# swiss-territorial-data-lab/proj-roadsurf

Hardware: AMD Instinct MI355X
Metric: tiles_per_sec_512x512x3 (higher is better)
Workload: dtype f16 hi + lo operand planes (22 significand bits, 3 MFMA products per product) / f32 accumulate; 1 GPU; Mask R-CNN R50-FPN inference, batch 16 of 512x512 3-band tiles per GPU (BASELINE configs[1]), 800x800 network input; seeded synthetic weights, saturated: 1000 proposals and 100 detections per tile; batch_per_gpu=16, lanes=2, lane_streams=independent, num_classes=2, weights=random

## Files before the change

### proj_roadsurf_amd/csrc/common.h

```cpp
#pragma once
#include <hip/hip_runtime.h>
#include <stdint.h>
#include <stdio.h>

typedef _Float16 half_t;
typedef _Float16 half4 __attribute__((ext_vector_type(4)));
typedef _Float16 half8 __attribute__((ext_vector_type(8)));
typedef float f32x4 __attribute__((ext_vector_type(4)));

#define RS_OK 0
#define RS_ERR_ARG -1
#define RS_ERR_HIP -2
#define RS_ERR_BLOB -3
#define RS_ERR_UNSUPPORTED -4

void rs_set_error(const char* fmt, ...);

#define RS_HIP(expr)                                                                       \
  do {                                                                                     \
    hipError_t _e = (expr);                                                                \
    if (_e != hipSuccess) {                                                                \
      rs_set_error("%s:%d: %s -> %s", __FILE__, __LINE__, #expr, hipGetErrorString(_e));   \
      return RS_ERR_HIP;                                                                   \
    }                                                                                      \
  } while (0)

#define RS_CHECK(cond, code, ...)  \
  do {                             \
    if (!(cond)) {                 \
      rs_set_error(__VA_ARGS__);   \
      return (code);               \
    }                              \
  } while (0)

static inline int cdiv(long long a, long long b) { return (int)((a + b - 1) / b); }

#if defined(__HIPCC__)
__device__ __forceinline__ float rs_fdiv(float a, float b) {
  const float y0 = __builtin_amdgcn_rcpf(b);
  const float e = __builtin_fmaf(-b, y0, 1.0f);
  const float y = __builtin_fmaf(e, y0, y0);
  const float q0 = a * y;
  const float r0 = __builtin_fmaf(-b, q0, a);
  const float q1 = __builtin_fmaf(r0, y, q0);
  const float r1 = __builtin_fmaf(-b, q1, a);
  const float q = __builtin_fmaf(r1, y, q1);
  const bool special = !(__builtin_fabsf(b) > 0.f && __builtin_fabsf(b) < __builtin_inff() && __builtin_fabsf(a) > 0.f && __builtin_fabsf(a) < __builtin_inff());
  return special ? a * y0 : q;
}

__device__ __forceinline__ unsigned rs_sat_bad(float f) { return !(__builtin_fabsf(f) <= 65504.f); }
__device__ __forceinline__ void rs_sat_flush(unsigned long long* sat, unsigned cnt) {
  if (sat != nullptr && cnt != 0u) atomicAdd(sat, (unsigned long long)cnt);
}
#endif

struct RsDebug {
  int conv_single_stage_nk = 4;
  int conv_persist = 0;
  int conv_tuned = 1;
  int conv_deep = 1;
  int conv_wide_px = 128;
  int wreg_dbg = 0;
  int wreg_waves = 2;
  int conv_wreg = 1;
  int conv_wide1x1 = 1;
  int stem_small_tile = 1;
  int deep_dbg = 0;
  int deconv_variant = 22;
  int fuse_mask_predictor = 1;
  int side_stream = 1;
  int narrow_roialign = 0;
  int use_glds = 1;
  int fuse_shortcut = 1;
  int fuse_stem = 1;
  int fuse_bneck = 1;
  int deep_tile_px = 1;
  int deep_tail = 1;
  int fuse_rpn_heads = 1;
  int merge_levels = 1;
  int graph_small = 1;
  int use_graph = 0;
  int train_roi_side = -1;
  int train_side = -1;
  int wgrad_target = 512;
  int wgrad_cb = 0;
  int select_debug = 0;
  int nms_debug = 0;
  int roi_window = 1;
  int roi_bwd_atomic = 0;
  int roi_order = 1;
  int poly_edge_cap = 0;
  int poly_vertex_cap = 0;
};
const RsDebug& rs_debug();
void rs_debug_reload();

struct ConvSeg {
  const half_t* in;
  const half_t* w;
  const float* bias;
  void* out;
  float* head_out;
  int Ho, Wo, in_Hp, in_Wp, out_Hp, out_Wp;
  int M;
  int tile0;
  long long in_lo, out_lo;
  const float* wscale;
};
#define RS_MAX_SEGS 5

struct ConvParams {
  const half_t* in;
  const half_t* w;
  const float* bias;
  void* out;
  const half_t* res;
  const half_t* up;
  const int* m_count;
  const int* koff;
  int m_mul;
  int M;
  int Ho, Wo;
  int in_Hp, in_Wp, in_Cs, in_off;
  int stride;
  int KH, KW, Cin;
  int Kpad;
  int Cout;
  int out_Hp, out_Wp, out_Cs, out_pad;
  int up_Hp, up_Wp, up_Cs, up_pad;
  int relu;
  int mode;
  int out_f32;
  const float* dot_w;
// ... 180 lines not shown
```

### proj_roadsurf_amd/csrc/conv_deep.hip

```cpp
#include "conv_tile.h"

namespace {

constexpr int BN = 256, NT = 512, MI = 4, WCH = 4;
constexpr int ASTAGE = 256 * 128, WSTAGE = BN * 128;
constexpr int W_BASE = 3 * ASTAGE;
constexpr int LDS_BYTES = 3 * ASTAGE + 2 * WSTAGE;

template <int DBG, bool TRAIN, int NJ, bool SPLIT>
__device__ __forceinline__ void conv_deep_tile(const ConvParams& p, char* smem, const half_t* g_in, const half_t* g_w, const float* g_bias, void* g_out,
                                               float* g_head_out, const int Ho, const int Wo, const int in_Hp, const int in_Wp, const int out_Hp, const int out_Wp,
                                               const int M, const int m0, const int n0, const int q, const long long in_lo, const long long out_lo,
                                               const float* g_wscale) {
  constexpr int APS = (NJ + 1) / 2;
  constexpr int WPX = NJ * 16;
  const int tid = threadIdx.x;
  const int lane = tid & 63;
  const int wave = __builtin_amdgcn_readfirstlane(tid >> 6);
  const int wpx = wave / WCH, wch = wave % WCH;
  (void)q;

  const int lrow = lane >> 3, lchk = lane & 7;
  const half_t* aptr[APS];
  const half_t* wptr[4];
// ... 203 lines not shown
      } else {
        __builtin_amdgcn_sched_barrier(0);
        asm volatile("s_waitcnt lgkmcnt(0)" ::: "memory");
      }
      sab = snext;
      __builtin_amdgcn_sched_barrier(0);
#pragma unroll
      for (int i = 0; i < MI; ++i)
#pragma unroll
        for (int j = 0; j < NJ; ++j)
          acc[i][j] = __builtin_amdgcn_mfma_f32_16x16x32_f16(wf1[i], xf0[j], acc[i][j], 0, 0, 0);
    }
#undef RS_RD_W
#undef RS_RD_X
#ifdef RS_SPLIT_PHASES
    ph_loop1 = __builtin_amdgcn_s_memtime();
    if (p.probe && lane == 0) {
      long long* o = p.probe + ((long long)q * 8 + wave) * 8;
      o[0] = (long long)ph_work; o[1] = (long long)ph_vm; o[2] = (long long)ph_bar; o[3] = nk;
      o[4] = (long long)(ph_loop0 - ph_entry); o[5] = (long long)(ph_loop1 - ph_loop0);
    }
#endif
  } else {
  reads0(0, 0);
  int abuf = 0;
  for (int t = 0; t < nk; ++t) {
    __builtin_amdgcn_sched_barrier(0);
    reads1(abuf, t & 1);
    __builtin_amdgcn_sched_barrier(0);
    asm volatile("s_waitcnt lgkmcnt(%0)" ::"n"(4 + NJ) : "memory");
    __builtin_amdgcn_sched_barrier(0);
#pragma unroll
    for (int i = 0; i < MI; ++i)
#pragma unroll
      for (int j = 0; j < NJ; ++j)
        acc[i][j] = __builtin_amdgcn_mfma_f32_16x16x32_f16(wf0[i], xf0[j], acc[i][j], 0, 0, 0);
    __builtin_amdgcn_sched_barrier(0);
    const int anext = abuf == 2 ? 0 : abuf + 1;
    if (t + 1 < nk) {
      asm volatile("s_waitcnt lgkmcnt(0)" ::: "memory");
      if (t + 2 < nk) asm volatile("s_waitcnt vmcnt(%0)" ::"n"(APS) : "memory");
      else asm volatile("s_waitcnt vmcnt(0)" ::: "memory");
      asm volatile("s_barrier" ::: "memory");
      __builtin_amdgcn_sched_barrier(0);
#ifndef RS_DEEP_LOCKSTEP
      if (wpx) {
#pragma unroll
        for (int i = 0; i < MI; ++i)
#pragma unroll
          for (int j = 0; j < NJ; ++j)
            acc[i][j] = __builtin_amdgcn_mfma_f32_16x16x32_f16(wf1[i], xf1[j], acc[i][j], 0, 0, 0);
        __builtin_amdgcn_sched_barrier(0);
      }
#endif
      if (t + 2 < nk) stage_w();
      if (t + 3 < nk) stage_a();
      reads0(anext, (t + 1) & 1);
#ifndef RS_DEEP_LOCKSTEP
      if (wpx) { abuf = anext; continue; }
#endif
    }
    else {
      __builtin_amdgcn_sched_barrier(0);
      asm volatile("s_waitcnt lgkmcnt(0)" ::: "memory");
    }
    abuf = anext;
    __builtin_amdgcn_sched_barrier(0);
#pragma unroll
    for (int i = 0; i < MI; ++i)
#pragma unroll
      for (int j = 0; j < NJ; ++j)
        acc[i][j] = __builtin_amdgcn_mfma_f32_16x16x32_f16(wf1[i], xf1[j], acc[i][j], 0, 0, 0);
  }
  }

#ifdef RS_CLOCK_PROBE
  if (p.probe && tid == 0) {
    p.probe[2 * q] = (long long)(__builtin_amdgcn_s_memtime() - pr_t0);
    p.probe[2 * q + 1] = (long long)(__builtin_amdgcn_s_memrealtime() - pr_r0);
  }
#endif
  const int crow = n0 + wch * 64 + fq * 16;
  const EpiRows<MI, SPLIT> rw = epi_rows<MI, SPLIT>(g_bias, g_wscale, crow);
  unsigned satc = 0;
  if (!TRAIN && p.head_w) {
    const half_t* hw = p.head_w + (long long)fi * 256 + wch * 64 + fq * 8;
    const half8 ha0 = *(const half8*)hw, ha1 = *(const half8*)(hw + 32);
    half8 hl0, hl1;
    if constexpr (SPLIT) { hl0 = *(const half8*)(hw + p.head_w_lo); hl1 = *(const half8*)(hw + p.head_w_lo + 32); }
    f32x4 hacc[NJ];
#pragma unroll
    for (int j = 0; j < NJ; ++j) {
      half8 b0, b1, l0, l1;
      const bool mv = m0 + wpx * WPX + j * 16 + fi < M;
      unsigned sath = 0;
#pragma unroll
      for (int i = 0; i < MI; ++i)
#pragma unroll
        for (int r = 0; r < 4; ++r) {
          float f;
          if constexpr (SPLIT) f = acc[i][j][r] * rw.wsc[i * 4 + r] + rw.bias[i * 4 + r];
          else f = acc[i][j][r] + rw.bias[i * 4 + r];
          if (p.relu) f = f > 0.f ? f : 0.f;
          sath += mv ? rs_sat_bad(f) : 0u;
          const HiLo s = split_round(clamp_h16(f));
          if (i < 2) { b0[i * 4 + r] = s.h; l0[i * 4 + r] = s.l; } else { b1[(i - 2) * 4 + r] = s.h; l1[(i - 2) * 4 + r] = s.l; }
        }
      rs_sat_flush(p.sat, sath);
      f32x4 a = f32x4{0.f, 0.f, 0.f, 0.f};
      a = __builtin_amdgcn_mfma_f32_16x16x32_f16(ha0, b0, a, 0, 0, 0);
      a = __builtin_amdgcn_mfma_f32_16x16x32_f16(ha1, b1, a, 0, 0, 0);
      if constexpr (SPLIT) {
        a = __builtin_amdgcn_mfma_f32_16x16x32_f16(ha0, l0, a, 0, 0, 0);
        a = __builtin_amdgcn_mfma_f32_16x16x32_f16(ha1, l1, a, 0, 0, 0);
        a = __builtin_amdgcn_mfma_f32_16x16x32_f16(hl0, b0, a, 0, 0, 0);
        a = __builtin_amdgcn_mfma_f32_16x16x32_f16(hl1, b1, a, 0, 0, 0);
      }
      hacc[j] = a;
    }
    asm volatile("s_barrier" ::: "memory");
    float* part = (float*)smem;
#pragma unroll
    for (int j = 0; j < NJ; ++j) *(f32x4*)(part + ((wch * 2 * WPX + wpx * WPX + j * 16 + fi) * 16 + fq * 4)) = hacc[j];
    __syncthreads();
    const int px = tid >> 1, oh = (tid & 1) * 8;
    const int m = m0 + px;
    if (px < 2 * WPX && m < M) {
      f32x4 s0 = f32x4{0.f, 0.f, 0.f, 0.f}, s1 = f32x4{0.f, 0.f, 0.f, 0.f};
      if constexpr (!SPLIT) { s0 = *(const f32x4*)(p.head_b + oh); s1 = *(const f32x4*)(p.head_b + oh + 4); }
#pragma unroll
      for (int w = 0; w < 4; ++w) {
        s0 += *(const f32x4*)(part + ((w * 2 * WPX + px) * 16 + oh));
        s1 += *(const f32x4*)(part + ((w * 2 * WPX + px) * 16 + oh + 4));
      }
      if constexpr (SPLIT) {
        s0 = s0 * *(const f32x4*)(p.head_scale + oh) + *(const f32x4*)(p.head_b + oh);
        s1 = s1 * *(const f32x4*)(p.head_scale + oh + 4) + *(const f32x4*)(p.head_b + oh + 4);
      }
      const Pix hp = pix_of(m, Wo, Ho);
      float* op = g_head_out + ((long long)(hp.n * Ho + hp.y) * Wo + hp.x) * 16 + oh;
      *(f32x4*)op = s0;
      *(f32x4*)(op + 4) = s1;
    }
    return;
  }
#pragma unroll
  for (int j = 0; j < NJ; ++j) {
    const int m = m0 + wpx * WPX + j * 16 + fi;
    if (m >= M) continue;
    const Pix px = pix_of(m, Wo, Ho);
    const long long opix = (long long)(px.n * out_Hp + px.y + p.out_pad) * out_Wp + px.x + p.out_pad;
    float v[4 * MI];
    epi_values<MI, NJ, TRAIN, SPLIT>(v, p, acc, j, rw, opix, crow, px.x, px.y, px.n);
    if (p.out_f32) epi_store_f32<MI>((float*)g_out + opix * p.out_Cs + crow, v);
    else epi_store_h16<MI, SPLIT>((half_t*)g_out + opix * p.out_Cs + crow, out_lo, v, [&](float f, float) { satc += rs_sat_bad(f); });
  }
  rs_sat_flush(p.sat, satc);
#ifdef RS_SPLIT_PHASES
  if constexpr (SPLIT) {
    const unsigned long long ph_issued = __builtin_amdgcn_s_memtime();
    asm volatile("s_waitcnt vmcnt(0)" ::: "memory");
    const unsigned long long ph_drained = __builtin_amdgcn_s_memtime();
    if (p.probe && lane == 0) {
      long long* o = p.probe + ((long long)q * 8 + wave) * 8;
      o[6] = (long long)(ph_issued - ph_loop1); o[7] = (long long)(ph_drained - ph_issued);
    }
  }
#endif
}


template <int DBG, bool TRAIN = false, int NJF = 8, bool SPLIT = false>
__global__ __launch_bounds__(NT) void conv_deep_kernel(const ConvParams p) {
  constexpr int BM = 32 * NJF;
  extern __shared__ __attribute__((aligned(16))) char smem[];
  int M = conv_rows(p);
  const int tiles_n = p.Cout / BN;
  const int ntiles = p.nseg ? p.seg_tiles : tiles_n * ((M + BM - 1) / BM);
  const int nfull = ntiles - p.tail_tiles;
  const int q = blockIdx.x;
  if (q >= nfull + 2 * p.tail_tiles) return;
  const half_t* g_in = p.in;
  const half_t* g_w = p.w;
  const float* g_bias = p.bias;
  void* g_out = p.out;
  float* g_head_out = p.head_out;
  long long in_lo = p.in_lo, out_lo = p.out_lo;
  const float* g_wscale = p.wscale;
  int Ho = p.Ho, Wo = p.Wo, in_Hp = p.in_Hp, in_Wp = p.in_Wp, out_Hp = p.out_Hp, out_Wp = p.out_Wp;
  int L, half = -1;
  if (q < nfull) {
    L = xcd_tile(q, nfull);
  } else {
    L = nfull + ((q - nfull) >> 1);
    half = (q - nfull) & 1;
  }
  if (p.nseg) {
    int t0 = 0;
#pragma unroll
    for (int i = 0; i < RS_MAX_SEGS; ++i)
      if (i < p.nseg && L >= p.seg[i].tile0) {
        g_in = p.seg[i].in; g_w = p.seg[i].w; g_bias = p.seg[i].bias; g_out = p.seg[i].out; g_head_out = p.seg[i].head_out;
        Ho = p.seg[i].Ho; Wo = p.seg[i].Wo; in_Hp = p.seg[i].in_Hp; in_Wp = p.seg[i].in_Wp;
        out_Hp = p.seg[i].out_Hp; out_Wp = p.seg[i].out_Wp; M = p.seg[i].M; t0 = p.seg[i].tile0;
        if constexpr (SPLIT) { in_lo = p.seg[i].in_lo; out_lo = p.seg[i].out_lo; g_wscale = p.seg[i].wscale; }
      }
    L -= t0;
  }
  const int n0 = (L % tiles_n) * BN;
  const int m0 = (L / tiles_n) * BM;
  if (half < 0 || NJF != 8) {
    conv_deep_tile<DBG, TRAIN, NJF, SPLIT>(p, smem, g_in, g_w, g_bias, g_out, g_head_out, Ho, Wo, in_Hp, in_Wp, out_Hp, out_Wp, M, m0, n0, q, in_lo, out_lo, g_wscale);
  } else {
    if (m0 + half * (BM / 2) >= M) return;
    conv_deep_tile<DBG, TRAIN, NJF == 8 ? 4 : NJF, SPLIT>(p, smem, g_in, g_w, g_bias, g_out, g_head_out, Ho, Wo, in_Hp, in_Wp, out_Hp, out_Wp, M, m0 + half * (BM / 2), n0, q, in_lo, out_lo, g_wscale);
  }
}

}

int rs_device_cu_count() {
  static int ncu[64] = {0};
  int dev = 0;
  if (hipGetDevice(&dev) != hipSuccess || dev < 0 || dev >= 64) return 256;
  if (!ncu[dev]) {
    int n = 0;
    if (hipDeviceGetAttribute(&n, hipDeviceAttributeMultiprocessorCount, dev) != hipSuccess || n <= 0) n = 256;
    ncu[dev] = n;
  }
  return ncu[dev];
}

static int deep_tail_tiles(long long tiles) {
  const int ncu = rs_device_cu_count();
  if (!rs_debug().deep_tail) return 0;
  const int r = (int)(tiles % ncu);
  return (r > 0 && 2 * r <= ncu) ? r : 0;
}

static int no_scratch(const void* kernel, const char* what) {
// ... 146 lines not shown
```

### proj_roadsurf_amd/csrc/conv_igemm.hip

```cpp
#include "conv_tile.h"

namespace {

template <int WPX, int WCH, int MI, int NJ>
struct Tile {
  static constexpr int NW = WPX * WCH;
  static constexpr int NT = NW * 64;
  static constexpr int BM = WPX * NJ * 16;
  static constexpr int BN = WCH * MI * 16;
  static constexpr int STAGE = (BM + BN) * 128;
  static constexpr int LDS = 2 * STAGE + 1024;
};

template <int WPX, int WCH, int MI, int NJ, bool SMALLC, bool GLDS, bool PERSIST, bool TRAIN = false, bool SPLIT = false, bool FWD = false>
__global__ __launch_bounds__(WPX* WCH * 64) void conv_igemm_kernel(const ConvParams p) {
  using T = Tile<WPX, WCH, MI, NJ>;
  constexpr int NW = T::NW, BM = T::BM, BN = T::BN;
  constexpr int PA = BM / (NW * 8);
  constexpr int PW = (BN + NW * 8 - 1) / (NW * 8);
  extern __shared__ __attribute__((aligned(16))) char smem[];

  const int tid = threadIdx.x;
  const int lane = tid & 63;
  const int wave = __builtin_amdgcn_readfirstlane(tid >> 6);
// ... 147 lines not shown
      if (PERSIST && t == 0 && stores_in_flight) {
        if (stores_in_flight == NJ * STORES_F16) asm volatile("s_waitcnt vmcnt(%0)" ::"n"(NJ * STORES_F16) : "memory");
        else if (stores_in_flight == NJ * STORES_F32) asm volatile("s_waitcnt vmcnt(%0)" ::"n"(NJ * STORES_F32) : "memory");
        else asm volatile("s_waitcnt vmcnt(0)" ::: "memory");
        asm volatile("s_waitcnt lgkmcnt(0)" ::: "memory");
        __builtin_amdgcn_s_barrier();
      } else {
        asm volatile("s_waitcnt vmcnt(0)" ::: "memory");
        __syncthreads();
      }
      if (nst == 2) {
        if (t + 1 < nk) {
          stage((gs + 1) & 1, t + 1, SMALLC ? 0 : next_off());
        } else if (PERSIST && q + G < ntiles) {
          setup_tile(q + G);
          kh = 0; kw = 0; c0 = 0;
          stage((gs + 1) & 1, 0, SMALLC ? 0 : next_off());
        }
      }
      const char* sb = smem + (nst == 2 ? (gs & 1) : 0) * T::STAGE;
      if constexpr (SPLIT && !SMALLC) {
        half8 wh[MI], wl[MI], xh[NJ], xl[NJ];
#pragma unroll
        for (int i = 0; i < MI; ++i) { wh[i] = *(const half8*)(sb + w_off[i] + c0_off); wl[i] = *(const half8*)(sb + w_off[i] + c1_off); }
#pragma unroll
        for (int j = 0; j < NJ; ++j) { xh[j] = *(const half8*)(sb + x_off[j] + c0_off); xl[j] = *(const half8*)(sb + x_off[j] + c1_off); }
#pragma unroll
        for (int i = 0; i < MI; ++i)
#pragma unroll
          for (int j = 0; j < NJ; ++j) mfma_split3(acc[i][j], wh[i], wl[i], xh[j], xl[j]);
      } else if constexpr (NJ == 8) {
        half8 wf0[MI], xf0[NJ], wf1[MI], xf1[NJ];
#pragma unroll
        for (int i = 0; i < MI; ++i) wf0[i] = *(const half8*)(sb + w_off[i] + c0_off);
#pragma unroll
        for (int j = 0; j < NJ; ++j) xf0[j] = *(const half8*)(sb + x_off[j] + c0_off);
#pragma unroll
        for (int i = 0; i < MI; ++i) wf1[i] = *(const half8*)(sb + w_off[i] + c1_off);
#pragma unroll
        for (int j = 0; j < NJ; ++j) xf1[j] = *(const half8*)(sb + x_off[j] + c1_off);
#pragma unroll
        for (int i = 0; i < MI; ++i)
#pragma unroll
          for (int j = 0; j < NJ; ++j)
            acc[i][j] = __builtin_amdgcn_mfma_f32_16x16x32_f16(wf0[i], xf0[j], acc[i][j], 0, 0, 0);
#pragma unroll
        for (int i = 0; i < MI; ++i)
#pragma unroll
          for (int j = 0; j < NJ; ++j)
            acc[i][j] = __builtin_amdgcn_mfma_f32_16x16x32_f16(wf1[i], xf1[j], acc[i][j], 0, 0, 0);
      } else {
#pragma unroll
        for (int kk = 0; kk < 2; ++kk) {
          const int co = kk ? c1_off : c0_off;
          half8 wf[MI], xf[NJ];
#pragma unroll
          for (int i = 0; i < MI; ++i) wf[i] = *(const half8*)(sb + w_off[i] + co);
#pragma unroll
          for (int j = 0; j < NJ; ++j) xf[j] = *(const half8*)(sb + x_off[j] + co);
#pragma unroll
          for (int i = 0; i < MI; ++i)
#pragma unroll
            for (int j = 0; j < NJ; ++j)
              acc[i][j] = __builtin_amdgcn_mfma_f32_16x16x32_f16(wf[i], xf[j], acc[i][j], 0, 0, 0);
        }
      }
      if (nst == 1 && t + 1 < nk) {
        __syncthreads();
        stage(0, t + 1, SMALLC ? 0 : next_off());
      }
      ++gs;
    }

    const int ch_local = wch * MI * 16 + fq * 4 * MI;
    const int crow = n0c + ch_local;
    int g = 0, cb = crow;
    if (p.mode != 0) { g = crow / p.Cout; cb = crow % p.Cout; }
    constexpr bool DGRAD_SPLIT = TRAIN && SPLIT;
    constexpr bool FWD_SPLIT = DGRAD_SPLIT && FWD;
    const EpiRows<MI, SPLIT> rw = epi_rows<MI, SPLIT>(DGRAD_SPLIT && !FWD_SPLIT ? p.wscale : p.bias, p.wscale, crow);
    int e_dy = 0;
    if constexpr (FWD_SPLIT) e_dy = split_tensor_exp(p.x_amax[0], p.x_amax[1]);
    else if constexpr (DGRAD_SPLIT) e_dy = split_tensor_exp(p.dy_amax[0], p.dy_amax[1]);
    float dotp[NJ];
    long long dot_idx[NJ];
#pragma unroll
    for (int j = 0; j < NJ; ++j) { dotp[j] = 0.f; dot_idx[j] = -1; }
#pragma unroll
    for (int j = 0; j < NJ; ++j) {
      const int m = m0c + wpx * NJ * 16 + j * 16 + fi;
      if (m >= M) continue;
      const Pix px = pix_of(m, p.Wo, p.Ho);
      const int x = px.x, y = px.y, n = px.n;
      int oy = y, ox = x;
      if (p.mode != 0) { oy = 2 * y + (g >> 1); ox = 2 * x + (g & 1); }
      else if (TRAIN && p.out_stride > 1) { oy = y * p.out_stride; ox = x * p.out_stride; }
      const long long opix = (long long)(n * p.out_Hp + oy + p.out_pad) * p.out_Wp + ox + p.out_pad;
      float v[4 * MI];
      if constexpr (DGRAD_SPLIT) {
        if constexpr (FWD_SPLIT) epi_values_fwd_split<MI, NJ>(v, p, acc, j, rw, e_dy, opix, cb, x, y, n);
        else epi_values_dgrad_split<MI, NJ>(v, p, acc, j, rw, e_dy, opix, cb, x, y, n);
        epi_store_f32<MI>((float*)p.out + opix * p.out_Cs + cb, v);
        continue;
      } else {
        epi_values<MI, NJ, TRAIN, SPLIT>(v, p, acc, j, rw, opix, cb, x, y, n);
      }
      if (p.mode == 2) {
        const int slot = p.dot_slot[n];
        const float* wv = p.dot_w + (long long)p.dot_cls[slot] * p.Cout + cb;
        float sdot = 0.f;
#pragma unroll
        for (int i = 0; i < MI; ++i) {
          const f32x4 w4 = *(const f32x4*)(wv + i * 4);
#pragma unroll
          for (int r = 0; r < 4; ++r) sdot += v[i * 4 + r] * w4[r];
        }
        dotp[j] = sdot;
        dot_idx[j] = (long long)slot * (4 * p.Ho * p.Wo) + (long long)oy * (2 * p.Wo) + ox;
      } else if (p.out_f32) {
        epi_store_f32<MI>((float*)p.out + opix * p.out_Cs + cb, v);
      } else {
        float scr = 0.f;
        epi_store_h16<MI, SPLIT>((half_t*)p.out + opix * p.out_Cs + cb, p.out_lo, v, [&](float, float f) { scr += __builtin_fabsf(f); });
        if (!(scr < 65504.f)) {
          unsigned c = 0;
#pragma unroll
          for (int e = 0; e < 4 * MI; ++e) c += rs_sat_bad(v[e]);
          rs_sat_flush(p.sat, c);
        }
      }
    }
    if (p.mode == 2) {
      float* red = (float*)smem;
      __syncthreads();
#pragma unroll
      for (int j = 0; j < NJ; ++j) {
        float v0 = dotp[j];
        v0 += __shfl_xor(v0, 16);
        v0 += __shfl_xor(v0, 32);
        dotp[j] = v0;
        if (wch > 0 && fq == 0) red[(((wch - 1) * WPX + wpx) * NJ + j) * 16 + fi] = v0;
      }
      __syncthreads();
      if (wch == 0 && fq == 0) {
#pragma unroll
        for (int j = 0; j < NJ; ++j) {
          float v0 = dotp[j];
#pragma unroll
          for (int c = 1; c < WCH; ++c) v0 += red[(((c - 1) * WPX + wpx) * NJ + j) * 16 + fi];
          if (dot_idx[j] >= 0) atomicAdd(p.dot_out + dot_idx[j], v0);
        }
      }
    }

    stores_in_flight = (p.mode != 2 && m0c + BM <= M) ? NJ * (p.out_f32 ? STORES_F32 : STORES_F16) : 0;
    if constexpr (!PERSIST) break;
    q += G;
    if (q >= ntiles) break;
    if (nst == 1) {
      setup_tile(q);
      kh = 0; kw = 0; c0 = 0;
      __syncthreads();
      stage(0, 0, SMALLC ? 0 : next_off());
    }
  }
}

template <int WPX, int WCH, int MI, int NJ, bool SMALLC, bool CAN_PERSIST>
int launch_variant(const ConvParams& p, hipStream_t stream, int use_glds) {
  using T = Tile<WPX, WCH, MI, NJ>;
  const int rows = p.Cout * (p.mode != 0 ? 4 : 1);
  const int tiles_n = cdiv(rows, T::BN);
  const int tiles_m = cdiv(p.M, T::BM);
  const long long nblk = (long long)tiles_n * tiles_m;
  RS_CHECK(nblk > 0 && nblk < (1ll << 31), RS_ERR_ARG, "conv: bad grid %lld", nblk);
  RS_CHECK(rows % T::BN == 0 || T::BN <= 16, RS_ERR_ARG, "conv: Cout rows %d not a multiple of tile %d", rows, T::BN);
  const int lds = (p.stages == 1 ? 1 : 2) * T::STAGE + 1024;
  int bpc = CAN_PERSIST ? p.persist : 0;
  if (bpc < 0) bpc = (160 * 1024) / lds < 1 ? 1 : (160 * 1024) / lds;
  const bool persistent = bpc > 0 && p.stages != 1 && p.mode != 2 && use_glds && nblk > 256ll * bpc &&
                          !(p.down || p.res32 || p.mask || p.out_stride > 1);
  const bool train = p.down || p.res32 || p.mask || p.out_stride > 1;
  const void* k;
  if (p.split) {
    RS_CHECK(use_glds > 0 && !train && p.wscale, RS_ERR_UNSUPPORTED, "conv: the split-operand mode needs LDS-DMA staging, the row scales and no training epilogue");
    k = (const void*)conv_igemm_kernel<WPX, WCH, MI, NJ, SMALLC, true, false, false, true>;
  } else if (train) {
    RS_CHECK(use_glds && !SMALLC, RS_ERR_UNSUPPORTED, "conv: training epilogue options need LDS-DMA staging and Cin >= 64");
    if constexpr (!SMALLC) k = (const void*)conv_igemm_kernel<WPX, WCH, MI, NJ, false, true, false, true>;
    else k = nullptr;
  } else if constexpr (CAN_PERSIST) {
    k = persistent ? (const void*)conv_igemm_kernel<WPX, WCH, MI, NJ, SMALLC, true, true>
                   : (use_glds ? (const void*)conv_igemm_kernel<WPX, WCH, MI, NJ, SMALLC, true, false>
                               : (const void*)conv_igemm_kernel<WPX, WCH, MI, NJ, SMALLC, false, false>);
  } else {
    k = use_glds ? (const void*)conv_igemm_kernel<WPX, WCH, MI, NJ, SMALLC, true, false>
                 : (const void*)conv_igemm_kernel<WPX, WCH, MI, NJ, SMALLC, false, false>;
  }
  static bool attr[5] = {false, false, false, false, false};
  const int ai = p.split ? 4 : (train ? 3 : (persistent ? 2 : (use_glds ? 1 : 0)));
  if (!attr[ai]) {
    RS_HIP(hipFuncSetAttribute(k, hipFuncAttributeMaxDynamicSharedMemorySize, T::LDS));
    attr[ai] = true;
  }
  const unsigned grid = (persistent && !p.split) ? 256u * (unsigned)bpc : (unsigned)nblk;
  ConvParams pc = p;
  void* args[] = {&pc};
  RS_HIP(hipLaunchKernel(k, dim3(grid), dim3(T::NT), args, lds, stream));
  return RS_OK;
}

template <int WPX, int WCH, int MI, int NJ, bool FWD = false>
// ... 244 lines not shown
```

### proj_roadsurf_amd/csrc/conv_tile.h

```cpp
#pragma once
#include <stdint.h>

#if defined(__HIPCC__)
#include "common.h"
#define CT_D __device__ __forceinline__
#else
#define CT_D inline
#endif

CT_D int xcd_tile(int q, int n) {
  const int qn = n >> 3, r = n & 7, x = q & 7;
  return (x < r ? x * (qn + 1) : r * (qn + 1) + (x - r) * qn) + (q >> 3);
}

CT_D int act_key(int row) { return row & 7; }
CT_D int w_key(int row, int blk) { return (row & 3) | ((int)(((unsigned)row / (unsigned)blk) & 1u) << 2); }
CT_D int src_chunk(int lchk, int key) { return lchk ^ key; }
CT_D int chunk_f16(int d) { return d * 8; }
CT_D long long chunk_split(int d, long long lo) { return (d & 3) * 8 + (d >> 2) * lo; }
CT_D int frag_row(int fi, int i, int blk) { return (fi >> 2) * blk + i * 4 + (fi & 3); }
CT_D int frag_off(int fq, int fkey, int kk) { return ((4 * kk + fq) ^ fkey) * 16; }

struct Pix { int x, y, n; };
CT_D Pix pix_of(int m, int Wo, int Ho) {
  const int t = m / Wo;
  return Pix{m % Wo, t % Ho, t / Ho};
}
CT_D Pix pix_add(int x0, int y0, int n0, int rx, int ry, int rn, int Wo, int Ho) {
  int x = x0 + rx;
  const int cx = x >= Wo;
  x -= cx ? Wo : 0;
  int y = y0 + ry + cx;
  const int cy = y >= Ho;
  y -= cy ? Ho : 0;
  return Pix{x, y, n0 + rn + cy};
}

#if !defined(CT_NO_F16)
#if !defined(__HIPCC__)
typedef _Float16 half_t;
#endif
CT_D float clamp_h16(float f) { return f > 65504.f ? 65504.f : (f < -65504.f ? -65504.f : f); }
CT_D float clamp_h16_pos(float f) { return f > 65504.f ? 65504.f : f; }
struct HiLo { half_t h, l; };
CT_D HiLo split_round(float f) {
  const half_t h = (half_t)f;
  return HiLo{h, (half_t)(f - (float)h)};
}
#endif

#if defined(__HIPCC__)
__device__ __forceinline__ void glds16(const half_t* g, char* lds_wave_base) {
  __builtin_amdgcn_global_load_lds((const __attribute__((address_space(1))) void*)g,
                                   (__attribute__((address_space(3))) void*)lds_wave_base, 16, 0, 0);
}

template <class P>
__device__ __forceinline__ int conv_rows(const P& p) {
  int M = p.M;
  if (p.m_count) {
    const long long mc = (long long)(*p.m_count) * p.m_mul;
    if (mc < M) M = (int)mc;
  }
  return M;
}

__device__ __forceinline__ void mfma_split3(f32x4& acc, const half8& wh, const half8& wl, const half8& xh, const half8& xl) {
  acc = __builtin_amdgcn_mfma_f32_16x16x32_f16(wh, xl, acc, 0, 0, 0);
  acc = __builtin_amdgcn_mfma_f32_16x16x32_f16(wh, xh, acc, 0, 0, 0);
  acc = __builtin_amdgcn_mfma_f32_16x16x32_f16(wl, xh, acc, 0, 0, 0);
}

__device__ __forceinline__ int split_tensor_exp(unsigned amax_bits, unsigned nonfinite) {
  if (nonfinite || amax_bits == 0) return 0;
  const int be = (int)(amax_bits >> 23);
  const int E = be ? be - 127 : (31 - __clz((int)amax_bits)) - 149;
  return 14 - E;
}

template <int MI, bool SPLIT>
struct EpiRows {
  float bias[4 * MI];
  float wsc[SPLIT ? 4 * MI : 1];
};
template <int MI, bool SPLIT>
__device__ __forceinline__ EpiRows<MI, SPLIT> epi_rows(const float* bias, const float* wscale, int crow) {
  EpiRows<MI, SPLIT> rw;
#pragma unroll
  for (int i = 0; i < MI; ++i) {
    const f32x4 b4 = *(const f32x4*)(bias + crow + i * 4);
    rw.bias[i * 4 + 0] = b4[0]; rw.bias[i * 4 + 1] = b4[1]; rw.bias[i * 4 + 2] = b4[2]; rw.bias[i * 4 + 3] = b4[3];
  }
  if constexpr (SPLIT) {
#pragma unroll
    for (int i = 0; i < MI; ++i) {
      const f32x4 s4 = *(const f32x4*)(wscale + crow + i * 4);
      rw.wsc[i * 4 + 0] = s4[0]; rw.wsc[i * 4 + 1] = s4[1]; rw.wsc[i * 4 + 2] = s4[2]; rw.wsc[i * 4 + 3] = s4[3];
    }
  }
  return rw;
}

template <int MI, int NJ, bool TRAIN, bool SPLIT>
__device__ __forceinline__ void epi_values(float (&v)[4 * MI], const ConvParams& p, const f32x4 (&acc)[MI][NJ], const int j, const EpiRows<MI, SPLIT>& rw,
                                           const long long opix, const int cb, const int x, const int y, const int n) {
#pragma unroll
  for (int i = 0; i < MI; ++i)
#pragma unroll
    for (int r = 0; r < 4; ++r) {
      if constexpr (SPLIT) v[i * 4 + r] = acc[i][j][r] * rw.wsc[i * 4 + r] + rw.bias[i * 4 + r];
      else v[i * 4 + r] = acc[i][j][r] + rw.bias[i * 4 + r];
    }
  auto add_h16 = [&](const half_t* a, const long long lo) {
#pragma unroll
    for (int i = 0; i < MI; ++i) {
      const half4 h = *(const half4*)(a + i * 4);
      if constexpr (SPLIT) {
        const half4 l = *(const half4*)(a + lo + i * 4);
#pragma unroll
        for (int r = 0; r < 4; ++r) v[i * 4 + r] += (float)h[r] + (float)l[r];
      } else {
#pragma unroll
        for (int r = 0; r < 4; ++r) v[i * 4 + r] += (float)h[r];
      }
    }
  };
  if (p.res) add_h16(p.res + opix * p.out_Cs + cb, p.res_lo);
  if (p.up) {
    const long long upix = (long long)(n * p.up_Hp + (y >> 1) + p.up_pad) * p.up_Wp + (x >> 1) + p.up_pad;
    add_h16(p.up + upix * p.up_Cs + cb, p.up_lo);
  }
  if (TRAIN && p.down) {
#pragma unroll
    for (int dd = 0; dd < 4; ++dd) {
      const long long dpix = (long long)(n * p.down_Hp + 2 * y + (dd >> 1) + p.down_pad) * p.down_Wp + 2 * x + (dd & 1) + p.down_pad;
      const half_t* dp = p.down + dpix * p.down_Cs + cb;
#pragma unroll
      for (int i = 0; i < MI; ++i) {
        const half4 h = *(const half4*)(dp + i * 4);
#pragma unroll
        for (int r = 0; r < 4; ++r) v[i * 4 + r] += (float)h[r];
      }
    }
  }
  if (TRAIN && p.res32) {
    const float* rp = p.res32 + opix * p.out_Cs + cb;
#pragma unroll
    for (int i = 0; i < MI; ++i) {
      const f32x4 h = *(const f32x4*)(rp + i * 4);
#pragma unroll
      for (int r = 0; r < 4; ++r) v[i * 4 + r] += h[r];
    }
  }
  if (TRAIN && p.mask) {
    const half_t* mp = p.mask + opix * p.out_Cs + cb;
#pragma unroll
    for (int i = 0; i < MI; ++i) {
      const half4 h = *(const half4*)(mp + i * 4);
#pragma unroll
      for (int r = 0; r < 4; ++r) v[i * 4 + r] = (float)h[r] > 0.f ? v[i * 4 + r] : 0.f;
    }
  }
  if (p.relu) {
#pragma unroll
    for (int e = 0; e < 4 * MI; ++e) v[e] = v[e] > 0.f ? v[e] : 0.f;
  }
}

template <int MI, int NJ>
__device__ __forceinline__ void epi_values_dgrad_split(float (&v)[4 * MI], const ConvParams& p, const f32x4 (&acc)[MI][NJ], const int j, const EpiRows<MI, true>& rw,
                                                       const int e_dy, const long long opix, const int cb, const int x, const int y, const int n) {
#pragma unroll
  for (int e = 0; e < 4 * MI; ++e) v[e] = ldexpf(acc[e >> 2][j][e & 3] * rw.wsc[e], -e_dy);
  auto add_f32 = [&](const float* a) {
#pragma unroll
    for (int i = 0; i < MI; ++i) {
      const f32x4 h = *(const f32x4*)(a + i * 4);
#pragma unroll
      for (int r = 0; r < 4; ++r) v[i * 4 + r] += h[r];
    }
  };
  if (p.res) add_f32((const float*)p.res + opix * p.out_Cs + cb);
  if (p.down) {
#pragma unroll
    for (int dd = 0; dd < 4; ++dd) {
      const long long dpix = (long long)(n * p.down_Hp + 2 * y + (dd >> 1) + p.down_pad) * p.down_Wp + 2 * x + (dd & 1) + p.down_pad;
      add_f32((const float*)p.down + dpix * p.down_Cs + cb);
    }
  }
  if (p.res32) add_f32(p.res32 + opix * p.out_Cs + cb);
  if (p.mask) {
    const float* mp = (const float*)p.mask + opix * p.out_Cs + cb;
#pragma unroll
    for (int i = 0; i < MI; ++i) {
      const f32x4 h = *(const f32x4*)(mp + i * 4);
#pragma unroll
      for (int r = 0; r < 4; ++r) v[i * 4 + r] = h[r] > 0.f ? v[i * 4 + r] : 0.f;
    }
  }
}

template <int MI, int NJ>
__device__ __forceinline__ void epi_values_fwd_split(float (&v)[4 * MI], const ConvParams& p, const f32x4 (&acc)[MI][NJ], const int j, const EpiRows<MI, true>& rw,
                                                     const int e_x, const long long opix, const int cb, const int x, const int y, const int n) {
#pragma unroll
  for (int e = 0; e < 4 * MI; ++e) v[e] = ldexpf(acc[e >> 2][j][e & 3] * rw.wsc[e], -e_x) + rw.bias[e];
  auto add_f32 = [&](const float* a) {
#pragma unroll
    for (int i = 0; i < MI; ++i) {
      const f32x4 h = *(const f32x4*)(a + i * 4);
#pragma unroll
      for (int r = 0; r < 4; ++r) v[i * 4 + r] += h[r];
    }
  };
  if (p.res) add_f32((const float*)p.res + opix * p.out_Cs + cb);
  if (p.up) {
    const long long upix = (long long)(n * p.up_Hp + (y >> 1) + p.up_pad) * p.up_Wp + (x >> 1) + p.up_pad;
    add_f32((const float*)p.up + upix * p.up_Cs + cb);
  }
  if (p.relu) {
#pragma unroll
    for (int e = 0; e < 4 * MI; ++e) v[e] = v[e] > 0.f ? v[e] : 0.f;
  }
}

template <int MI>
__device__ __forceinline__ void epi_store_f32(float* op, const float (&v)[4 * MI]) {
#pragma unroll
  for (int i = 0; i < MI; ++i) *(f32x4*)(op + i * 4) = f32x4{v[i * 4], v[i * 4 + 1], v[i * 4 + 2], v[i * 4 + 3]};
}

template <int MI, bool SPLIT, class F>
__device__ __forceinline__ void epi_store_h16(half_t* op, const long long out_lo, const float (&v)[4 * MI], F&& count) {
  constexpr int W = MI % 2 == 0 ? 8 : 4;
  typedef _Float16 hvec __attribute__((ext_vector_type(W)));
#pragma unroll
  for (int c = 0; c < 4 * MI; c += W) {
    hvec h, l;
#pragma unroll
    for (int r = 0; r < W; ++r) {
      const float f = clamp_h16(v[c + r]);
      count(v[c + r], f);
      const HiLo s = split_round(f);
      h[r] = s.h;
      l[r] = s.l;
    }
    *(hvec*)(op + c) = h;
    if constexpr (SPLIT) *(hvec*)(op + out_lo + c) = l;
  }
}
#endif
```

Baseline: 955.9 tiles/s.

## Streamline conv epilogues with wave-uniform saturation screening and scalarized args

Reworks the convolution epilogues in the deep and implicit-GEMM kernels. A wave-wide ballot screens for values outside the f16 range, so clamping and counting run only when some lane saturates. ReLU becomes a single v_max against an SGPR floor instead of a branch, and epilogue parameters are pinned in scalar registers. Pixel coordinates advance incrementally instead of recomputing a division per j, and residual loads use the global address space. The intent is to cut VALU work and register pressure in the epilogue. The inline-asm register pinning and the divergent slow path add some risk.

```diff
diff --git a/proj_roadsurf_amd/csrc/common.h b/proj_roadsurf_amd/csrc/common.h
--- a/proj_roadsurf_amd/csrc/common.h
+++ b/proj_roadsurf_amd/csrc/common.h
@@ -2,6 +2,7 @@
 #include <hip/hip_runtime.h>
 #include <stdint.h>
 #include <stdio.h>
+#include "sat_bad.h"
 
 typedef _Float16 half_t;
 typedef _Float16 half4 __attribute__((ext_vector_type(4)));
@@ -49,7 +50,6 @@
   return special ? a * y0 : q;
 }
 
-__device__ __forceinline__ unsigned rs_sat_bad(float f) { return !(__builtin_fabsf(f) <= 65504.f); }
 __device__ __forceinline__ void rs_sat_flush(unsigned long long* sat, unsigned cnt) {
   if (sat != nullptr && cnt != 0u) atomicAdd(sat, (unsigned long long)cnt);
 }
diff --git a/proj_roadsurf_amd/csrc/conv_deep.hip b/proj_roadsurf_amd/csrc/conv_deep.hip
--- a/proj_roadsurf_amd/csrc/conv_deep.hip
+++ b/proj_roadsurf_amd/csrc/conv_deep.hip
@@ -309,7 +309,7 @@
 #endif
   const int crow = n0 + wch * 64 + fq * 16;
   const EpiRows<MI, SPLIT> rw = epi_rows<MI, SPLIT>(g_bias, g_wscale, crow);
-  unsigned satc = 0;
+  const EpiArgs ea = epi_args(p);
   if (!TRAIN && p.head_w) {
     const half_t* hw = p.head_w + (long long)fi * 256 + wch * 64 + fq * 8;
     const half8 ha0 = *(const half8*)hw, ha1 = *(const half8*)(hw + 32);
@@ -320,20 +320,27 @@
     for (int j = 0; j < NJ; ++j) {
       half8 b0, b1, l0, l1;
       const bool mv = m0 + wpx * WPX + j * 16 + fi < M;
-      unsigned sath = 0;
+      float f[4 * MI];
 #pragma unroll
       for (int i = 0; i < MI; ++i)
 #pragma unroll
         for (int r = 0; r < 4; ++r) {
-          float f;
-          if constexpr (SPLIT) f = acc[i][j][r] * rw.wsc[i * 4 + r] + rw.bias[i * 4 + r];
-          else f = acc[i][j][r] + rw.bias[i * 4 + r];
-          if (p.relu) f = f > 0.f ? f : 0.f;
-          sath += mv ? rs_sat_bad(f) : 0u;
-          const HiLo s = split_round(clamp_h16(f));
+          if constexpr (SPLIT) f[i * 4 + r] = acc[i][j][r] * rw.wsc[i * 4 + r] + rw.bias[i * 4 + r];
+          else f[i * 4 + r] = acc[i][j][r] + rw.bias[i * 4 + r];
+        }
+#pragma unroll
+      for (int e = 0; e < 4 * MI; ++e) f[e] = relu_f32(ea.floor, f[e]);
+      if (__builtin_amdgcn_ballot_w64(sat_screen(f)) != 0ull) {
+        const unsigned c = sat_clamp_count(f);
+        rs_sat_flush(ea.sat, mv ? c : 0u);
+      }
+#pragma unroll
+      for (int i = 0; i < MI; ++i)
+#pragma unroll
+        for (int r = 0; r < 4; ++r) {
+          const HiLo s = split_round(f[i * 4 + r]);
           if (i < 2) { b0[i * 4 + r] = s.h; l0[i * 4 + r] = s.l; } else { b1[(i - 2) * 4 + r] = s.h; l1[(i - 2) * 4 + r] = s.l; }
         }
-      rs_sat_flush(p.sat, sath);
       f32x4 a = f32x4{0.f, 0.f, 0.f, 0.f};
       a = __builtin_amdgcn_mfma_f32_16x16x32_f16(ha0, b0, a, 0, 0, 0);
       a = __builtin_amdgcn_mfma_f32_16x16x32_f16(ha1, b1, a, 0, 0, 0);
@@ -371,18 +378,18 @@
     }
     return;
   }
+  PixWalk pw = pix_walk(m0 + wpx * WPX + fi, Wo, Ho);
 #pragma unroll
   for (int j = 0; j < NJ; ++j) {
-    const int m = m0 + wpx * WPX + j * 16 + fi;
-    if (m >= M) continue;
-    const Pix px = pix_of(m, Wo, Ho);
-    const long long opix = (long long)(px.n * out_Hp + px.y + p.out_pad) * out_Wp + px.x + p.out_pad;
+    if (j) pix_next(pw);
+    if (m0 + wpx * WPX + j * 16 + fi >= M) continue;
+    const Pix px = pw.p;
+    const long long opix = (long long)(px.n * out_Hp + px.y + ea.out_pad) * out_Wp + px.x + ea.out_pad;
     float v[4 * MI];
-    epi_values<MI, NJ, TRAIN, SPLIT>(v, p, acc, j, rw, opix, crow, px.x, px.y, px.n);
-    if (p.out_f32) epi_store_f32<MI>((float*)g_out + opix * p.out_Cs + crow, v);
-    else epi_store_h16<MI, SPLIT>((half_t*)g_out + opix * p.out_Cs + crow, out_lo, v, [&](float f, float) { satc += rs_sat_bad(f); });
-  }
-  rs_sat_flush(p.sat, satc);
+    epi_values<MI, NJ, TRAIN, SPLIT>(v, p, ea, acc, j, rw, opix, crow, px.x, px.y, px.n);
+    if (ea.out_f32) epi_store_f32<MI>((float*)g_out + opix * ea.out_Cs + crow, v);
+    else epi_store_h16<MI, SPLIT>((half_t*)g_out + opix * ea.out_Cs + crow, out_lo, v, ea.sat);
+  }
 #ifdef RS_SPLIT_PHASES
   if constexpr (SPLIT) {
     const unsigned long long ph_issued = __builtin_amdgcn_s_memtime();
diff --git a/proj_roadsurf_amd/csrc/conv_igemm.hip b/proj_roadsurf_amd/csrc/conv_igemm.hip
--- a/proj_roadsurf_amd/csrc/conv_igemm.hip
+++ b/proj_roadsurf_amd/csrc/conv_igemm.hip
@@ -253,20 +253,21 @@
     int e_dy = 0;
     if constexpr (FWD_SPLIT) e_dy = split_tensor_exp(p.x_amax[0], p.x_amax[1]);
     else if constexpr (DGRAD_SPLIT) e_dy = split_tensor_exp(p.dy_amax[0], p.dy_amax[1]);
+    const EpiArgs ea = epi_args(p);
     float dotp[NJ];
     long long dot_idx[NJ];
 #pragma unroll
     for (int j = 0; j < NJ; ++j) { dotp[j] = 0.f; dot_idx[j] = -1; }
+    PixWalk pw = pix_walk(m0c + wpx * NJ * 16 + fi, p.Wo, p.Ho);
 #pragma unroll
     for (int j = 0; j < NJ; ++j) {
-      const int m = m0c + wpx * NJ * 16 + j * 16 + fi;
-      if (m >= M) continue;
-      const Pix px = pix_of(m, p.Wo, p.Ho);
-      const int x = px.x, y = px.y, n = px.n;
+      if (j) pix_next(pw);
+      if (m0c + wpx * NJ * 16 + j * 16 + fi >= M) continue;
+      const int x = pw.p.x, y = pw.p.y, n = pw.p.n;
       int oy = y, ox = x;
       if (p.mode != 0) { oy = 2 * y + (g >> 1); ox = 2 * x + (g & 1); }
       else if (TRAIN && p.out_stride > 1) { oy = y * p.out_stride; ox = x * p.out_stride; }
-      const long long opix = (long long)(n * p.out_Hp + oy + p.out_pad) * p.out_Wp + ox + p.out_pad;
+      const long long opix = (long long)(n * p.out_Hp + oy + ea.out_pad) * p.out_Wp + ox + ea.out_pad;
       float v[4 * MI];
       if constexpr (DGRAD_SPLIT) {
         if constexpr (FWD_SPLIT) epi_values_fwd_split<MI, NJ>(v, p, acc, j, rw, e_dy, opix, cb, x, y, n);
@@ -274,7 +275,7 @@
         epi_store_f32<MI>((float*)p.out + opix * p.out_Cs + cb, v);
         continue;
       } else {
-        epi_values<MI, NJ, TRAIN, SPLIT>(v, p, acc, j, rw, opix, cb, x, y, n);
+        epi_values<MI, NJ, TRAIN, SPLIT>(v, p, ea, acc, j, rw, opix, cb, x, y, n);
       }
       if (p.mode == 2) {
         const int slot = p.dot_slot[n];
@@ -288,17 +289,10 @@
         }
         dotp[j] = sdot;
         dot_idx[j] = (long long)slot * (4 * p.Ho * p.Wo) + (long long)oy * (2 * p.Wo) + ox;
-      } else if (p.out_f32) {
-        epi_store_f32<MI>((float*)p.out + opix * p.out_Cs + cb, v);
+      } else if (ea.out_f32) {
+        epi_store_f32<MI>((float*)p.out + opix * ea.out_Cs + cb, v);
       } else {
-        float scr = 0.f;
-        epi_store_h16<MI, SPLIT>((half_t*)p.out + opix * p.out_Cs + cb, p.out_lo, v, [&](float, float f) { scr += __builtin_fabsf(f); });
-        if (!(scr < 65504.f)) {
-          unsigned c = 0;
-#pragma unroll
-          for (int e = 0; e < 4 * MI; ++e) c += rs_sat_bad(v[e]);
-          rs_sat_flush(p.sat, c);
-        }
+        epi_store_h16<MI, SPLIT>((half_t*)p.out + opix * ea.out_Cs + cb, ea.out_lo, v, ea.sat);
       }
     }
     if (p.mode == 2) {
diff --git a/proj_roadsurf_amd/csrc/conv_tile.h b/proj_roadsurf_amd/csrc/conv_tile.h
--- a/proj_roadsurf_amd/csrc/conv_tile.h
+++ b/proj_roadsurf_amd/csrc/conv_tile.h
@@ -1,5 +1,6 @@
 #pragma once
 #include <stdint.h>
+#include "sat_bad.h"
 
 #if defined(__HIPCC__)
 #include "common.h"
@@ -36,18 +37,59 @@
   return Pix{x, y, n0 + rn + cy};
 }
 
+struct PixWalk {
+  Pix p, step;
+  int Wo, Ho;
+};
+CT_D PixWalk pix_walk(int m_first, int Wo, int Ho) { return PixWalk{pix_of(m_first, Wo, Ho), pix_of(16, Wo, Ho), Wo, Ho}; }
+CT_D void pix_next(PixWalk& w) { w.p = pix_add(w.p.x, w.p.y, w.p.n, w.step.x, w.step.y, w.step.n, w.Wo, w.Ho); }
+
+template <int N>
+CT_D bool sat_screen(const float (&v)[N]) {
+  bool bad = false;
+#if defined(__HIPCC__)
+#pragma unroll
+#endif
+  for (int e = 0; e < N; ++e) bad |= rs_sat_bad(v[e]) != 0u;
+  return bad;
+}
+CT_D unsigned relu_floor(bool relu) { return relu ? 0u : 0x7fc00000u; }
+CT_D float relu_f32(unsigned floor, float f) {
+#if defined(__HIP_DEVICE_COMPILE__)
+  float r;
+  asm("v_max_f32_e64 %0, %2, %1" : "=v"(r) : "s"(floor), "v"(f));
+  return r;
+#else
+  return floor == 0u ? (f > 0.f ? f : 0.f) : f;
+#endif
+}
+
+CT_D float clamp_h16(float f) { return f > 65504.f ? 65504.f : (f < -65504.f ? -65504.f : f); }
+CT_D float clamp_h16_pos(float f) { return f > 65504.f ? 65504.f : f; }
+
 #if !defined(CT_NO_F16)
 #if !defined(__HIPCC__)
 typedef _Float16 half_t;
 #endif
-CT_D float clamp_h16(float f) { return f > 65504.f ? 65504.f : (f < -65504.f ? -65504.f : f); }
-CT_D float clamp_h16_pos(float f) { return f > 65504.f ? 65504.f : f; }
 struct HiLo { half_t h, l; };
 CT_D HiLo split_round(float f) {
   const half_t h = (half_t)f;
   return HiLo{h, (half_t)(f - (float)h)};
 }
 #endif
+
+template <int N>
+CT_D unsigned sat_clamp_count(float (&v)[N]) {
+  unsigned c = 0;
+#if defined(__HIPCC__)
+#pragma unroll
+#endif
+  for (int e = 0; e < N; ++e) {
+    c += rs_sat_bad(v[e]);
+    v[e] = clamp_h16(v[e]);
+  }
+  return c;
+}
 
 #if defined(__HIPCC__)
 __device__ __forceinline__ void glds16(const half_t* g, char* lds_wave_base) {
@@ -98,12 +140,31 @@
       rw.wsc[i * 4 + 0] = s4[0]; rw.wsc[i * 4 + 1] = s4[1]; rw.wsc[i * 4 + 2] = s4[2]; rw.wsc[i * 4 + 3] = s4[3];
     }
   }
+#pragma unroll
+  for (int i = 0; i < MI; ++i) {
+    asm volatile("" ::"v"(rw.bias[i * 4]), "v"(rw.bias[i * 4 + 1]), "v"(rw.bias[i * 4 + 2]), "v"(rw.bias[i * 4 + 3]));
+    if constexpr (SPLIT) asm volatile("" ::"v"(rw.wsc[i * 4]), "v"(rw.wsc[i * 4 + 1]), "v"(rw.wsc[i * 4 + 2]), "v"(rw.wsc[i * 4 + 3]));
+  }
   return rw;
 }
 
+struct EpiArgs {
+  const half_t *res, *up;
+  long long res_lo, up_lo, out_lo;
+  unsigned long long* sat;
+  int out_Cs, out_pad, up_Hp, up_Wp, up_pad, up_Cs, out_f32;
+  unsigned floor;
+};
+__device__ __forceinline__ EpiArgs epi_args(const ConvParams& p) {
+  EpiArgs a{p.res, p.up, p.res_lo, p.up_lo, p.out_lo, p.sat, p.out_Cs, p.out_pad, p.up_Hp, p.up_Wp, p.up_pad, p.up_Cs, p.out_f32, relu_floor(p.relu != 0)};
+  asm volatile("" : "+s"(a.res), "+s"(a.up), "+s"(a.res_lo), "+s"(a.up_lo), "+s"(a.out_lo), "+s"(a.sat));
+  asm volatile("" : "+s"(a.out_Cs), "+s"(a.out_pad), "+s"(a.up_Hp), "+s"(a.up_Wp), "+s"(a.up_pad), "+s"(a.up_Cs), "+s"(a.out_f32), "+s"(a.floor));
+  return a;
+}
+
 template <int MI, int NJ, bool TRAIN, bool SPLIT>
-__device__ __forceinline__ void epi_values(float (&v)[4 * MI], const ConvParams& p, const f32x4 (&acc)[MI][NJ], const int j, const EpiRows<MI, SPLIT>& rw,
-                                           const long long opix, const int cb, const int x, const int y, const int n) {
+__device__ __forceinline__ void epi_values(float (&v)[4 * MI], const ConvParams& p, const EpiArgs& a, const f32x4 (&acc)[MI][NJ], const int j,
+                                           const EpiRows<MI, SPLIT>& rw, const long long opix, const int cb, const int x, const int y, const int n) {
 #pragma unroll
   for (int i = 0; i < MI; ++i)
 #pragma unroll
@@ -111,12 +172,13 @@
       if constexpr (SPLIT) v[i * 4 + r] = acc[i][j][r] * rw.wsc[i * 4 + r] + rw.bias[i * 4 + r];
       else v[i * 4 + r] = acc[i][j][r] + rw.bias[i * 4 + r];
     }
-  auto add_h16 = [&](const half_t* a, const long long lo) {
-#pragma unroll
-    for (int i = 0; i < MI; ++i) {
-      const half4 h = *(const half4*)(a + i * 4);
+  auto add_h16 = [&](const half_t* a0, const long long lo) {
+    const auto* ap = (const __attribute__((address_space(1))) half_t*)a0;
+#pragma unroll
+    for (int i = 0; i < MI; ++i) {
+      const half4 h = *(const __attribute__((address_space(1))) half4*)(ap + i * 4);
       if constexpr (SPLIT) {
-        const half4 l = *(const half4*)(a + lo + i * 4);
+        const half4 l = *(const __attribute__((address_space(1))) half4*)(ap + lo + i * 4);
 #pragma unroll
         for (int r = 0; r < 4; ++r) v[i * 4 + r] += (float)h[r] + (float)l[r];
       } else {
@@ -125,10 +187,10 @@
       }
     }
   };
-  if (p.res) add_h16(p.res + opix * p.out_Cs + cb, p.res_lo);
-  if (p.up) {
-    const long long upix = (long long)(n * p.up_Hp + (y >> 1) + p.up_pad) * p.up_Wp + (x >> 1) + p.up_pad;
-    add_h16(p.up + upix * p.up_Cs + cb, p.up_lo);
+  if (a.res) add_h16(a.res + opix * a.out_Cs + cb, a.res_lo);
+  if (a.up) {
+    const long long upix = (long long)(n * a.up_Hp + (y >> 1) + a.up_pad) * a.up_Wp + (x >> 1) + a.up_pad;
+    add_h16(a.up + upix * a.up_Cs + cb, a.up_lo);
   }
   if (TRAIN && p.down) {
 #pragma unroll
@@ -161,10 +223,8 @@
       for (int r = 0; r < 4; ++r) v[i * 4 + r] = (float)h[r] > 0.f ? v[i * 4 + r] : 0.f;
     }
   }
-  if (p.relu) {
-#pragma unroll
-    for (int e = 0; e < 4 * MI; ++e) v[e] = v[e] > 0.f ? v[e] : 0.f;
-  }
+#pragma unroll
+  for (int e = 0; e < 4 * MI; ++e) v[e] = relu_f32(a.floor, v[e]);
 }
 
 template <int MI, int NJ>
@@ -230,23 +290,30 @@
   for (int i = 0; i < MI; ++i) *(f32x4*)(op + i * 4) = f32x4{v[i * 4], v[i * 4 + 1], v[i * 4 + 2], v[i * 4 + 3]};
 }
 
-template <int MI, bool SPLIT, class F>
-__device__ __forceinline__ void epi_store_h16(half_t* op, const long long out_lo, const float (&v)[4 * MI], F&& count) {
+template <int MI, bool SPLIT>
+__device__ __forceinline__ void epi_store_h16(half_t* op, const long long out_lo, float (&v)[4 * MI], unsigned long long* sat) {
   constexpr int W = MI % 2 == 0 ? 8 : 4;
   typedef _Float16 hvec __attribute__((ext_vector_type(W)));
-#pragma unroll
-  for (int c = 0; c < 4 * MI; c += W) {
-    hvec h, l;
-#pragma unroll
-    for (int r = 0; r < W; ++r) {
-      const float f = clamp_h16(v[c + r]);
-      count(v[c + r], f);
-      const HiLo s = split_round(f);
-      h[r] = s.h;
-      l[r] = s.l;
-    }
-    *(hvec*)(op + c) = h;
-    if constexpr (SPLIT) *(hvec*)(op + out_lo + c) = l;
-  }
-}
-#endif
+  auto round_store = [&](const float (&u)[4 * MI]) {
+#pragma unroll
+    for (int c = 0; c < 4 * MI; c += W) {
+      hvec h, l;
+#pragma unroll
+      for (int r = 0; r < W; ++r) {
+        const HiLo s = split_round(u[c + r]);
+        h[r] = s.h;
+        l[r] = s.l;
+      }
+      *(hvec*)(op + c) = h;
+      if constexpr (SPLIT) *(hvec*)(op + out_lo + c) = l;
+    }
+  };
+  if (__builtin_amdgcn_ballot_w64(sat_screen(v)) != 0ull) {
+    const unsigned c = sat_clamp_count(v);
+    round_store(v);
+    rs_sat_flush(sat, c);
+  } else {
+    round_store(v);
+  }
+}
+#endif
diff --git a/proj_roadsurf_amd/csrc/sat_bad.h b/proj_roadsurf_amd/csrc/sat_bad.h
--- /dev/null
+++ b/proj_roadsurf_amd/csrc/sat_bad.h
@@ -0,0 +1,7 @@
+#pragma once
+#if defined(__HIPCC__)
+#define RS_SAT_FN __host__ __device__ inline __attribute__((always_inline))
+#else
+#define RS_SAT_FN inline
+#endif
+RS_SAT_FN unsigned rs_sat_bad(float f) { return !(__builtin_fabsf(f) <= 65504.f); }
```

Result: no change. 958.2 tiles/s, median of 6 (+0.2%).
